# ashvardanian/StringZilla

Hardware: AMD Instinct MI355X
Metric: DP cell-updates/s (GCUPS) on 1M-pair Levenshtein batch (higher is better)
Workload: dtype u32 bit-vectors (u64 results)

## Files before the change

### stringzilla_amd/csrc/hip/device_common.hpp

```cpp
#pragma once
#include <hip/hip_runtime.h>
#include <stdint.h>

#include "kernels.h"

namespace szs_hip {

using u8 = uint8_t;
using u32 = uint32_t;
using u64 = uint64_t;
using i32 = int32_t;
using i64 = int64_t;

constexpr u32 wave_size_k = 64;

constexpr int device_slots_k = 64;
inline int device_slot() {
    int device = 0;
    if (hipGetDevice(&device) != hipSuccess) (void)hipGetLastError(), device = 0;
    return device < 0 || device >= device_slots_k ? 0 : device;
}
inline int cached(int const *slot) { return __atomic_load_n(slot, __ATOMIC_RELAXED); }
inline void remember(int *slot, int value) { __atomic_store_n(slot, value, __ATOMIC_RELAXED); }

__device__ __forceinline__ u32 wave_max_u32(u32 value) {
#pragma unroll
    for (int offset = 32; offset >= 1; offset >>= 1) {
        u32 const other = (u32)__shfl_xor((int)value, offset, 64);
        value = other > value ? other : value;
    }
    return value;
}

struct text_stream_t {
    u32 const *aligned_base;
    u32 byte_shift;
    u32 valid_dwords;

    __device__ __forceinline__ text_stream_t(u64 address, u32 length) {
        aligned_base = reinterpret_cast<u32 const *>(address & ~(u64)3);
        byte_shift = (u32)(address & 3);
        valid_dwords = length ? (byte_shift + length + 3) / 4 : 0;
    }

    __device__ __forceinline__ u32 raw(u32 dword_index) const {
        return dword_index < valid_dwords ? aligned_base[dword_index] : 0u;
    }

    __device__ __forceinline__ u32 raw_clamped(u32 dword_index) const {
        return aligned_base[dword_index < valid_dwords ? dword_index : valid_dwords - 1];
    }

    __device__ __forceinline__ u32 splice(u32 raw_low, u32 raw_high) const {
        return __builtin_amdgcn_alignbyte(raw_high, raw_low, byte_shift);
    }

    __device__ __forceinline__ static u32 symbol(u32 symbols, int step) { return (symbols >> (8 * step)) & 0xFFu; }
};

struct text_stream_backward_t {
    u32 const *aligned_base;
    u32 byte_shift;
    u32 valid_dwords;
    u32 top_dword;

    __device__ __forceinline__ text_stream_backward_t(u64 address, u32 length) {
        aligned_base = reinterpret_cast<u32 const *>(address & ~(u64)3);
        u64 const top = (address & 3) + (u64)length;
        byte_shift = (u32)(top & 3);
        valid_dwords = length ? (u32)((top + 3) / 4) : 0;
        top_dword = (u32)(top / 4);
    }

    __device__ __forceinline__ u32 raw(u32 back) const {
        u32 const dword_index = top_dword - back;
        return dword_index < valid_dwords ? aligned_base[dword_index] : 0u;
    }

    __device__ __forceinline__ u32 splice(u32 raw_high, u32 raw_low) const {
        return __builtin_amdgcn_alignbyte(raw_high, raw_low, byte_shift);
    }

    __device__ __forceinline__ static u32 symbol(u32 symbols, int step) { return (symbols >> (8 * (3 - step))) & 0xFFu; }
};

}
```

### stringzilla_amd/csrc/hip/lev_myers.hip

```cpp
#include "myers_core.hpp"

#define SZS_PAIR_RULE_FN __host__ __device__ static inline
#include "pair_rule.h"

#include <cstdlib>

namespace szs_hip {

#ifndef SZS_MYERS_PACK_QUERIES
#define SZS_MYERS_PACK_QUERIES 1
#endif
#ifndef SZS_MYERS_PAIR_RULES
#define SZS_MYERS_PAIR_RULES 1
#endif

#ifndef SZS_MYERS_SHORT_TEXT_DWORDS
#define SZS_MYERS_SHORT_TEXT_DWORDS 2
#endif


__device__ __forceinline__ u32 bits_in_word(u32 from, u32 to, int w) {
    u32 const low = from > 32u * w ? from : 32u * w, high = to < 32u * w + 32u ? to : 32u * w + 32u;
    if (low >= high) return 0u;
    return (high - low == 32u ? ~0u : (1u << (high - low)) - 1u) << (low - 32u * w);
}

template <int words_, int text_dwords_, bool runes_, bool paired_ = false>
__device__ __forceinline__ void myers_workgroup(u32 *peq, u32 *keys, szs_string_ref_t const query,
                                                szs_string_ref_t const *__restrict__ candidates, u32 candidates_count,
                                                u32 candidate_block, u64 *__restrict__ results, u64 results_row_stride,
                                                int symmetric, szs_ref_guard_t const &guard, u32 alphabet = 0,
                                                u32 *claimed_rows = nullptr, u32 blocks_here = 1, szs_string_ref_t const second = {}) {
    static_assert(!paired_ || !runes_, "query pairs are a byte-kernel shape");
    constexpr int rows = runes_ ? rune_slots_k : byte_rows_k;
    using layout = peq_layout<words_, rows>;
    if (guard.enabled && (!ref_is_current(guard, 0, query) || (paired_ && !ref_is_current(guard, 0, second)))) {
        if (threadIdx.x == 0) *guard.stale = guard.sequence;
        return;
    }
    u32 const first_length = query.length, second_length = paired_ ? second.length : 0u;
    u32 const query_length = paired_ ? first_length + second_length : first_length;
    u32 const used_rows = paired_ ? query_length + 2u : query_length;
    u32 const pad = 32u * words_ - used_rows;
    u32 const second_row = pad + first_length + 2u;

    for (int i = threadIdx.x; i < layout::total_dwords; i += 256) peq[i] = 0;
    if constexpr (runes_) {
        if (alphabet) {
            for (u32 i = threadIdx.x; i <= alphabet; i += 256) keys[i] = 0;
            if (threadIdx.x == 0) *claimed_rows = 0;
        }
        else
            for (int i = threadIdx.x; i < rune_slots_k; i += 256) keys[i] = rune_slot_empty_k;
    }
    __syncthreads();
    if (runes_ && alphabet) {
        u32 const *pattern = reinterpret_cast<u32 const *>(query.address);
        for (u32 i = threadIdx.x; i < query_length; i += 256) {
            u32 const id = pattern[i];
            if (atomicCAS(&keys[id], 0u, ~0u) == 0u) keys[id] = atomicAdd(claimed_rows, 1u) + 1;
        }
        __syncthreads();
        for (u32 i = threadIdx.x; i < query_length; i += 256) {
            u32 const position = pad + i;
            atomicOr(&peq[layout::dword_index((int)keys[pattern[i]], (int)(position >> 5))], 1u << (position & 31));
        }
    }
    else if constexpr (runes_) {
        u32 const *pattern = reinterpret_cast<u32 const *>(query.address);
        for (u32 i = threadIdx.x; i < query_length; i += 256) {
            u32 const rune = pattern[i];
            u32 slot = rune_slot_hash(rune);
            for (;;) {
                u32 const previous = atomicCAS(&keys[slot], rune_slot_empty_k, rune);
                if (previous == rune_slot_empty_k || previous == rune) break;
                slot = (slot + 1) & (rune_slots_k - 1);
            }
            u32 const position = pad + i;
            atomicOr(&peq[layout::dword_index((int)slot, (int)(position >> 5))], 1u << (position & 31));
        }
    }
    else {
        u8 const *pattern = reinterpret_cast<u8 const *>(query.address);
        for (u32 i = threadIdx.x; i < first_length; i += 256) {
            u32 const position = pad + i;
            atomicOr(&peq[layout::dword_index(pattern[i], (int)(position >> 5))], 1u << (position & 31));
        }
        if constexpr (paired_) {
            u8 const *above = reinterpret_cast<u8 const *>(second.address);
            for (u32 i = threadIdx.x; i < second_length; i += 256) {
                u32 const position = second_row + i;
                atomicOr(&peq[layout::dword_index(above[i], (int)(position >> 5))], 1u << (position & 31));
            }
        }
    }
    __syncthreads();
    pattern_pair_t<words_> boundary;
    if constexpr (paired_) {
#pragma unroll
        for (int w = 0; w < words_; ++w) {
            boundary.separators[w] = bits_in_word(second_row - 2u, second_row, w);
            boundary.tops[w] = first_length ? bits_in_word(second_row - 3u, second_row - 2u, w) : 0u;
        }
    }

#pragma unroll 1
    for (u32 block_step = 0; block_step < blocks_here; ++block_step) {
    u32 const candidate_slot = (candidate_block - block_step) * SZS_CANDIDATES_PER_WORKGROUP + threadIdx.x;
    bool live = candidate_slot < candidates_count;
    szs_string_ref_t candidate = {0, 0, 0};
    if (live) candidate = candidates[candidate_slot];
    if (live && guard.enabled && !ref_is_current(guard, 1, candidate)) {
        *guard.stale = guard.sequence;
        live = false;
    }
    if ((symmetric & SZS_LAYOUT_SYMMETRIC) && candidate.index > query.index) live = false;
    u32 const text_length = live ? candidate.length : 0;
    u32 const longest_in_wave = wave_max_u32(text_length);
    u32 const shortest_in_wave = ~wave_max_u32(live ? ~text_length : 0u);

    u32 vp[words_], vn[words_];
#pragma unroll
    for (int w = 0; w < words_; ++w) {
        vp[w] = bits_in_word(pad, 32u * words_, w) & ~(paired_ ? boundary.separators[w] : 0u);
        vn[w] = 0;
    }

    auto take = [&](u32 symbol) {
        u32 eq[words_];
        load_match_masks<words_, rows>(peq, !runes_ ? symbol : alphabet ? keys[symbol] : find_rune_slot(keys, symbol), eq);
        if constexpr (paired_) myers_column<words_>(vp, vn, eq, boundary);
        else myers_column<words_>(vp, vn, eq);
    };

    u32 column = 0;
    if constexpr (runes_) {
        u32 const *const runes = reinterpret_cast<u32 const *>(candidate.address);
        auto quad_at = [&](u32 index) -> uint4 {
            return index < text_length ? *reinterpret_cast<uint4 const *>(runes + index) : make_uint4(0, 0, 0, 0);
        };
        if (4 <= shortest_in_wave && longest_in_wave) {
            uint4 ahead = quad_at(0);
            for (; column + 4 <= shortest_in_wave; column += 4) {
                uint4 const now = ahead;
                ahead = quad_at(column + 4);
                take(now.x), take(now.y), take(now.z), take(now.w);
            }
        }
#pragma unroll 1
        for (; column < longest_in_wave; ++column)
            if (column < text_length) take(runes[column]);
    }
    else {
        u64 const safe_address = text_length ? candidate.address : first_length || !paired_ ? query.address : second.address;
        text_stream_t text(safe_address, text_length);
        if (!text_length) text.valid_dwords = query_length ? 1 : 0;
        u32 raw_low = text.raw(0);
        u32 dword = 0;
        constexpr u32 columns_per_iteration = 4 * text_dwords_;
#ifndef SZS_MYERS_CLAMPED_READS
#define SZS_MYERS_CLAMPED_READS(TEXT_DWORDS) ((TEXT_DWORDS) == 1)
#endif
        constexpr bool clamped_reads = SZS_MYERS_CLAMPED_READS(text_dwords_);
        if (columns_per_iteration <= shortest_in_wave && longest_in_wave && query_length) {
            u32 ahead[text_dwords_];
#pragma unroll
            for (int d = 0; d < text_dwords_; ++d) ahead[d] = clamped_reads ? text.raw_clamped(1 + d) : text.raw(1 + d);
            for (; column + columns_per_iteration <= shortest_in_wave;
                 column += columns_per_iteration, dword += text_dwords_) {
                u32 symbols[text_dwords_];
                symbols[0] = text.splice(raw_low, ahead[0]);
#pragma unroll
                for (int d = 1; d < text_dwords_; ++d) symbols[d] = text.splice(ahead[d - 1], ahead[d]);
                raw_low = ahead[text_dwords_ - 1];
#pragma unroll
                for (int d = 0; d < text_dwords_; ++d)
                    ahead[d] = clamped_reads ? text.raw_clamped(dword + text_dwords_ + 1 + d)
                                             : text.raw(dword + text_dwords_ + 1 + d);
#pragma unroll
                for (int step = 0; step < 4 * text_dwords_; ++step) take((symbols[step / 4] >> (8 * (step % 4))) & 0xFFu);
            }
        }
#ifndef SZS_MYERS_MID_LOOP
#define SZS_MYERS_MID_LOOP 0
#endif
        if constexpr (SZS_MYERS_MID_LOOP && text_dwords_ > 1) {
            if (column + 4 <= shortest_in_wave && longest_in_wave && query_length) {
                u32 ahead_one = text.raw(dword + 1);
#pragma unroll 1
                for (; column + 4 <= shortest_in_wave; column += 4, ++dword) {
                    u32 const symbols = text.splice(raw_low, ahead_one);
                    raw_low = ahead_one;
                    ahead_one = text.raw(dword + 2);
#pragma unroll
                    for (int step = 0; step < 4; ++step) take((symbols >> (8 * step)) & 0xFFu);
                }
            }
        }
        if (column < longest_in_wave) {
            u32 next = text.raw(dword + 1);
#pragma unroll 1
            for (; column < longest_in_wave; column += 4, ++dword) {
                u32 const after = text.raw(dword + 2);
                u32 const symbols = text.splice(raw_low, next);
                raw_low = next, next = after;
#pragma unroll
                for (int step = 0; step < 4; ++step)
                    if (column + step < text_length) take((symbols >> (8 * step)) & 0xFFu);
            }
        }
    }

    if (live && paired_) {
        u32 first = text_length, above = text_length;
#pragma unroll
        for (int w = 0; w < words_; ++w) {
            u32 const mine = bits_in_word(pad, pad + first_length, w), theirs = bits_in_word(second_row, 32u * words_, w);
            first += (u32)__builtin_popcount(vp[w] & mine) - (u32)__builtin_popcount(vn[w] & mine);
            above += (u32)__builtin_popcount(vp[w] & theirs) - (u32)__builtin_popcount(vn[w] & theirs);
        }
        bool const transposed = (symmetric & SZS_LAYOUT_TRANSPOSED) != 0;
        u64 const one = transposed ? candidate.index : query.index, two = transposed ? candidate.index : second.index;
        u64 const one_column = transposed ? query.index : candidate.index, two_column = transposed ? second.index : candidate.index;
        results[one * results_row_stride + one_column] = first;
        results[two * results_row_stride + two_column] = above;
    }
    else if (live) {
        u32 distance = text_length;
#pragma unroll
        for (int w = 0; w < words_; ++w) distance += (u32)__builtin_popcount(vp[w]) - (u32)__builtin_popcount(vn[w]);
        bool const transposed = (symmetric & SZS_LAYOUT_TRANSPOSED) != 0;
        u64 const row = transposed ? candidate.index : query.index, column = transposed ? query.index : candidate.index;
        results[row * results_row_stride + column] = distance;
        if ((symmetric & SZS_LAYOUT_SYMMETRIC) && candidate.index != query.index)
            results[column * results_row_stride + row] = distance;
    }
    }
}

#ifndef SZS_WORK_BLOCK_MAJOR
#define SZS_WORK_BLOCK_MAJOR 1
#endif
__device__ __forceinline__ void myers_work_item(u32 candidate_blocks, u32 &query_slot, u32 &candidate_block) {
#if SZS_WORK_BLOCK_MAJOR
    u32 const queries_count = gridDim.x / candidate_blocks;
    query_slot = blockIdx.x % queries_count;
    candidate_block = candidate_blocks - 1 - blockIdx.x / queries_count;
#else
    query_slot = blockIdx.x / candidate_blocks;
    candidate_block = candidate_blocks - 1 - blockIdx.x % candidate_blocks;
#endif
}

#ifndef SZS_MYERS_LONG_WAVES
#define SZS_MYERS_LONG_WAVES 2
#endif
template <int words_>
__global__ __launch_bounds__(256, SZS_MYERS_LONG_WAVES) void levenshtein_myers_long_kernel(szs_string_ref_t const *__restrict__ queries,
                                                                      szs_string_ref_t const *__restrict__ candidates,
                                                                      u32 candidates_count, u32 candidate_blocks,
                                                                      u64 *__restrict__ results, u64 results_row_stride,
                                                                      int symmetric, szs_ref_guard_t guard) {
    __shared__ __attribute__((aligned(16))) u32 peq[peq_layout<words_>::total_dwords];
    u32 query_slot, candidate_block;
    myers_work_item(candidate_blocks, query_slot, candidate_block);
    myers_workgroup<words_, 1, false>(peq, nullptr, queries[query_slot], candidates, candidates_count, candidate_block,
                                      results, results_row_stride, symmetric, guard);
}

__device__ __forceinline__ u64 fused_offset(void const *offsets, u32 wide, u64 index) {
    return wide ? static_cast<u64 const *>(offsets)[index] : (u64) static_cast<u32 const *>(offsets)[index];
}

__device__ __forceinline__ void fused_sort_side(szs_plan_side_t const &side, u32 is_query_side, u32 choose_rule, u32 sequence, u32 *ready,
                                                u32 second_ready, u32 withhold, szs_fused_side_report_t *report, u32 *histogram ,
                                                szs_string_ref_t *staged ) {
    constexpr u32 per_thread = SZS_FUSED_MOST_STRINGS / 256;
    u32 const tid = threadIdx.x, lane = tid & 63u, wave = tid >> 6, count = side.count;
    bool const one_pass = count <= SZS_FUSED_MOST_STRINGS;
    __shared__ u32 wave_bins[4], wave_longest[4], wave_status[4];
    __shared__ unsigned long long wave_symbols[4], wave_bands_systolic[4], wave_bands_chain[4], wave_squares[4];
    __shared__ u32 rule_words[256];

    u64 const began = wall_clock64();
    for (u32 bin = tid; bin < SZS_FUSED_BINS; bin += 256) histogram[bin] = 0;
    u64 from[per_thread], to[per_thread];
#pragma unroll
    for (u32 k = 0; k < per_thread; ++k) {
        u32 const i = tid + k * 256;
        from[k] = to[k] = 0;
        if (one_pass && i < count) from[k] = fused_offset(side.offsets, side.wide, i), to[k] = fused_offset(side.offsets, side.wide, (u64)i + 1);
    }
    __syncthreads();
    u32 bins[per_thread];
    u32 status = 0, longest = 0;
    u64 symbols = 0, bands_systolic = 0, bands_chain = 0, squares = 0;
    auto count_in = [&](u64 first, u64 last) -> u32 {
        if (last < first) return status |= SZS_PLAN_STATUS_DESCENDING, ~0u;
        if (last - first > 0xFFFFFFFFull) return status |= SZS_PLAN_STATUS_OVERFLOW, ~0u;
        u32 const length = (u32)(last - first);
        symbols += length, squares += (u64)length * length, longest = length > longest ? length : longest;
        bands_systolic += length ? (length + SZS_SYSTOLIC_BAND_ROWS - 1) / SZS_SYSTOLIC_BAND_ROWS : 1;
        bands_chain += length ? (length + SZS_MYERS_CHAIN_BAND_ROWS - 1) / SZS_MYERS_CHAIN_BAND_ROWS : 1;
        u32 const bin = length < SZS_FUSED_BINS - 1 ? length : SZS_FUSED_BINS - 1;
        atomicAdd(&histogram[bin], 1u);
        return bin;
    };
    if (one_pass) {
#pragma unroll
        for (u32 k = 0; k < per_thread; ++k) {
            bins[k] = ~0u;
            if (tid + k * 256 < count) bins[k] = count_in(from[k], to[k]);
        }
    }
    else {
#pragma unroll 1
        for (u32 first = 0; first < count; first += 1024) {
            u64 some_from[4], some_to[4];
#pragma unroll
            for (u32 k = 0; k < 4; ++k) {
                u32 const i = first + tid + k * 256;
                some_from[k] = some_to[k] = 0;
                if (i < count) some_from[k] = fused_offset(side.offsets, side.wide, i), some_to[k] = fused_offset(side.offsets, side.wide, (u64)i + 1);
            }
#pragma unroll
            for (u32 k = 0; k < 4; ++k)
                if (first + tid + k * 256 < count) (void)count_in(some_from[k], some_to[k]);
        }
    }
    if (tid == 0) report->ticks[0] = (u32)began, report->ticks[1] = (u32)(wall_clock64() - began);
#pragma unroll
    for (int offset = 32; offset >= 1; offset >>= 1) {
        status |= (u32)__shfl_xor((int)status, offset, 64);
        u32 const other = (u32)__shfl_xor((int)longest, offset, 64);
        longest = other > longest ? other : longest;
    }
    if (lane == 0) wave_status[wave] = status, wave_longest[wave] = longest;
    __syncthreads();
    u32 mine[4], sum = 0;
#pragma unroll
    for (u32 k = 0; k < 4; ++k) mine[k] = histogram[4 * tid + k], sum += mine[k];
    u32 inclusive = sum;
#pragma unroll
    for (int offset = 1; offset < 64; offset <<= 1) {
        u32 const other = (u32)__shfl_up((int)inclusive, offset, 64);
        if (lane >= (u32)offset) inclusive += other;
    }
    if (lane == 63) wave_bins[wave] = inclusive;
    __syncthreads();
    status = wave_status[0] | wave_status[1] | wave_status[2] | wave_status[3];
    longest = wave_longest[0];
#pragma unroll
    for (u32 w = 1; w < 4; ++w) longest = wave_longest[w] > longest ? wave_longest[w] : longest;
    u32 running = inclusive - sum;
    for (u32 w = 0; w < wave; ++w) running += wave_bins[w];
#pragma unroll
    for (u32 k = 0; k < 4; ++k) histogram[4 * tid + k] = running, running += mine[k];
    __syncthreads();
    if (tid == 0) report->ticks[2] = (u32)(wall_clock64() - began);
    u32 const blank = status || (is_query_side && longest > 32u * SZS_MYERS_SHORT_WORDS);
    if (one_pass) {
#pragma unroll
        for (u32 k = 0; k < per_thread; ++k) {
            u32 const i = tid + k * 256;
            if (i >= count) continue;
            szs_string_ref_t ref;
            ref.address = status ? side.base : side.base + from[k], ref.length = blank ? 0u : (u32)(to[k] - from[k]), ref.index = i;
            staged[status ? i : atomicAdd(&histogram[bins[k]], 1u)] = ref;
        }
        __syncthreads();
        for (u32 position = tid; position < count; position += 256) {
            szs_string_ref_t const ref = staged[position];
            side.ascending[position] = ref, side.descending[count - 1 - position] = ref;
        }
    }
    u32 const pair_slots = szs_pair_slots(count), pair_seconds = szs_pair_seconds(count);
    bool const choosing = choose_rule && one_pass && pair_seconds;
    if (choosing) {
        constexpr u32 strides = 256 / SZS_PAIR_RULE_CANDIDATES;
        u32 me = tid;
        asm volatile("" : "+v"(me));
        u32 const rule = szs_pair_rule_candidate(me % SZS_PAIR_RULE_CANDIDATES, pair_seconds);
        u32 words = 0;
        if (me < strides * SZS_PAIR_RULE_CANDIDATES) {
#pragma unroll 4
            for (u32 slot = me / SZS_PAIR_RULE_CANDIDATES; slot < pair_seconds; slot += strides)
                words += szs_pair_slot_words(staged[count - 1 - slot].length,
                                             staged[count - 1 - szs_pair_second_rank(rule, slot, pair_slots, pair_seconds)].length);
        }
        rule_words[me] = words;
    }
    if (!one_pass) {
#pragma unroll 1
        for (u32 first = 0; first < count; first += 1024) {
            u64 some_from[4], some_to[4];
#pragma unroll
            for (u32 k = 0; k < 4; ++k) {
                u32 const i = first + tid + k * 256;
                some_from[k] = some_to[k] = 0;
                if (i < count) some_from[k] = fused_offset(side.offsets, side.wide, i), some_to[k] = fused_offset(side.offsets, side.wide, (u64)i + 1);
            }
#pragma unroll
            for (u32 k = 0; k < 4; ++k) {
                u32 const i = first + tid + k * 256;
                if (i >= count) continue;
                u32 const length = status ? 0u : (u32)(some_to[k] - some_from[k]);
                szs_string_ref_t ref;
                ref.address = status ? side.base : side.base + some_from[k], ref.length = blank ? 0u : length, ref.index = i;
                u32 const position = status ? i : atomicAdd(&histogram[length < SZS_FUSED_BINS - 1 ? length : SZS_FUSED_BINS - 1], 1u);
                side.ascending[position] = ref, side.descending[count - 1 - position] = ref;
            }
        }
    }
    __syncthreads();
    if (tid == 0) report->ticks[3] = (u32)(wall_clock64() - began);
    u32 pairing = 0;
    if (choosing && wave == 0) {
        constexpr u32 strides = 256 / SZS_PAIR_RULE_CANDIDATES;
        u32 key = ~0u;
        if (lane < SZS_PAIR_RULE_CANDIDATES) {
            u32 total = 0;
#pragma unroll
            for (u32 k = 0; k < strides; ++k) total += rule_words[lane + k * SZS_PAIR_RULE_CANDIDATES];
            key = (total << 5) | lane;
        }
#pragma unroll
        for (int offset = 16; offset >= 1; offset >>= 1) {
            u32 const other = (u32)__shfl_xor((int)key, offset, 64);
            key = other < key ? other : key;
        }
        pairing = szs_pair_rule_candidate(key & 31u, pair_seconds);
    }
    if (tid == 0) {
        if (!withhold) {
            if (is_query_side)
                __hip_atomic_store(reinterpret_cast<u64 *>(ready), ((u64)pairing << 32) | sequence, __ATOMIC_RELEASE, __HIP_MEMORY_SCOPE_AGENT);
            else
                __hip_atomic_store(ready, sequence, __ATOMIC_RELEASE, __HIP_MEMORY_SCOPE_AGENT);
            if (second_ready) __hip_atomic_store(ready + 32, sequence, __ATOMIC_RELAXED, __HIP_MEMORY_SCOPE_AGENT);
        }
        report->ticks[4] = (u32)(wall_clock64() - began);
    }
#pragma unroll
    for (int offset = 32; offset >= 1; offset >>= 1) {
        symbols += ((u64)(u32)__shfl_xor((int)(u32)(symbols >> 32), offset, 64) << 32) | (u32)__shfl_xor((int)(u32)symbols, offset, 64);
        squares += ((u64)(u32)__shfl_xor((int)(u32)(squares >> 32), offset, 64) << 32) | (u32)__shfl_xor((int)(u32)squares, offset, 64);
        bands_systolic += ((u64)(u32)__shfl_xor((int)(u32)(bands_systolic >> 32), offset, 64) << 32) | (u32)__shfl_xor((int)(u32)bands_systolic, offset, 64);
        bands_chain += ((u64)(u32)__shfl_xor((int)(u32)(bands_chain >> 32), offset, 64) << 32) | (u32)__shfl_xor((int)(u32)bands_chain, offset, 64);
    }
    if (lane == 0) wave_symbols[wave] = symbols, wave_bands_systolic[wave] = bands_systolic, wave_bands_chain[wave] = bands_chain, wave_squares[wave] = squares;
    if (tid <= SZS_PLAN_RANK_SAMPLES) {
        u32 const rank = (u32)((u64)tid * (count ? count - 1 : 0) / SZS_PLAN_RANK_SAMPLES);
        report->rank_lengths[tid] = status || !count ? 0u : one_pass ? staged[rank].length : side.ascending[rank].length;
    }
    __syncthreads();
    if (tid == 0) {
        report->status = status, report->blank = blank, report->pairing = pairing;
        report->stats.count = count, report->stats.longest = longest;
        report->stats.symbols = wave_symbols[0] + wave_symbols[1] + wave_symbols[2] + wave_symbols[3];
        report->stats.bands_systolic = wave_bands_systolic[0] + wave_bands_systolic[1] + wave_bands_systolic[2] + wave_bands_systolic[3];
        report->stats.bands_chain = wave_bands_chain[0] + wave_bands_chain[1] + wave_bands_chain[2] + wave_bands_chain[3];
        report->squares = wave_squares[0] + wave_squares[1] + wave_squares[2] + wave_squares[3];
        report->sequence = sequence;
    }
}

__device__ __forceinline__ bool fused_prologue(szs_fused_plan_t const &plan, u32 *scratch, u32 &pairing) {
    __shared__ __attribute__((aligned(16))) szs_string_ref_t staged[SZS_FUSED_MOST_STRINGS];
    for (u32 s = 0; s < (plan.symmetric ? 1u : 2u); ++s)
        if (blockIdx.x == s % gridDim.x) {
            fused_sort_side(plan.side[s], s == 0, SZS_MYERS_PAIR_RULES && SZS_MYERS_PACK_QUERIES && s == 0 && !plan.symmetric && plan.blocks_per_group == 1,
                            plan.sequence, plan.ready + 32 * s, plan.symmetric, plan.withhold, plan.report + s, scratch, staged);
            __syncthreads();
        }
    __shared__ u32 unpublished[2], published_high[2];
    if (threadIdx.x < 2) {
        u32 polls = 0;
        u64 word;
        bool published;
        while (!(published = (u32)(word = __hip_atomic_load(reinterpret_cast<u64 const *>(plan.ready + 32 * threadIdx.x), __ATOMIC_RELAXED,
                                                             __HIP_MEMORY_SCOPE_AGENT)) == plan.sequence) &&
               ++polls < plan.poll_budget)
            __builtin_amdgcn_s_sleep(8);
        unpublished[threadIdx.x] = !published, published_high[threadIdx.x] = (u32)(word >> 32);
    }
    __syncthreads();
    pairing = (u32)__builtin_amdgcn_readfirstlane((int)published_high[0]);
    if (unpublished[0] | unpublished[1]) {
        if (threadIdx.x == 0) __hip_atomic_store(plan.gave_up, plan.sequence, __ATOMIC_RELAXED, __HIP_MEMORY_SCOPE_SYSTEM);
        return false;
    }
    return true;
}

#ifndef SZS_MYERS_SHORT_WAVES
#define SZS_MYERS_SHORT_WAVES 1
#endif
constexpr u32 szs_myers_pair_words_k = SZS_PAIR_WORDS_MOST;
template <bool runes_, bool merged_, bool fused_ = false>
__device__ __forceinline__ void myers_short_body(
    szs_string_ref_t const *__restrict__ queries, szs_string_ref_t const *__restrict__ candidates, u32 candidates_count,
    u32 candidate_blocks, u64 *__restrict__ results, u64 results_row_stride, int symmetric, szs_ref_guard_t guard, u32 alphabet,
    u32 blocks_per_group, szs_fused_plan_t const *fused = nullptr) {
    constexpr bool pairs = fused_ && !merged_ && SZS_MYERS_PACK_QUERIES;
    __shared__ __attribute__((aligned(16))) u32 peq[peq_layout<pairs ? szs_myers_pair_words_k : 8, runes_ ? rune_slots_k : byte_rows_k>::total_dwords];
    u32 pairing = 0;
    if constexpr (fused_) {
        static_assert(peq_layout<8, byte_rows_k>::total_dwords >= SZS_FUSED_BINS, "the sort's histogram borrows the masks' LDS");
        if (!fused_prologue(*fused, peq, pairing)) return;
    }
    __shared__ u32 slot_keys[runes_ ? rune_slots_k : 1];
    __shared__ u32 claimed_rows;
    extern __shared__ u32 rows_of_ids[];
    u32 *const keys = runes_ && alphabet ? rows_of_ids : slot_keys;
    u32 query_slot, candidate_group;
    myers_work_item(candidate_blocks, query_slot, candidate_group);
    u32 const all_blocks = (candidates_count + SZS_CANDIDATES_PER_WORKGROUP - 1) / SZS_CANDIDATES_PER_WORKGROUP;
    u32 const first_block = merged_ ? candidate_group * blocks_per_group : candidate_group;
    u32 const blocks_here = !merged_ ? 1u : all_blocks - first_block < blocks_per_group ? all_blocks - first_block : blocks_per_group;
    u32 const candidate_block = first_block + blocks_here - 1;
    szs_string_ref_t query = queries[query_slot];
    if constexpr (fused_) {
        query.address = ((u64)(u32)__builtin_amdgcn_readfirstlane((int)(u32)(query.address >> 32)) << 32) |
                        (u32)__builtin_amdgcn_readfirstlane((int)(u32)query.address);
// ... 1232 lines not shown
```

### stringzilla_amd/csrc/hip/myers_core.hpp

```cpp
#pragma once
#include "device_common.hpp"

namespace szs_hip {

constexpr int byte_rows_k = 256;
constexpr int rune_slots_k = 512;
constexpr u32 rune_slot_empty_k = ~0u;

template <int words_, int rows_ = byte_rows_k>
struct peq_layout {
    static constexpr int chunk_words = words_ >= 3 ? 4 : words_;
    static constexpr int chunks = (words_ + chunk_words - 1) / chunk_words;
    static constexpr int total_dwords = chunks * rows_ * chunk_words;
    __device__ static constexpr int dword_index(int row, int w) {
        return ((w / chunk_words) * rows_ + row) * chunk_words + (w % chunk_words);
    }
};

__device__ __forceinline__ u32 rune_slot_hash(u32 rune) { return (rune * 2654435761u) >> 23; }
__device__ __forceinline__ u32 find_rune_slot(u32 const *keys, u32 rune) {
    u32 slot = rune_slot_hash(rune);
    for (;;) {
        u32 const key = keys[slot];
        if (key == rune || key == rune_slot_empty_k) return slot;
        slot = (slot + 1) & (rune_slots_k - 1);
    }
}

template <int words_, int rows_>
__device__ __forceinline__ void load_match_masks(u32 const *peq, u32 symbol, u32 (&eq)[words_]) {
    using layout = peq_layout<words_, rows_>;
    if constexpr (layout::chunk_words == 4) {
        uint4 const *rows = reinterpret_cast<uint4 const *>(peq);
#pragma unroll
        for (int chunk = 0; chunk < layout::chunks; ++chunk) {
            uint4 const row = rows[chunk * rows_ + symbol];
            if (chunk * 4 + 0 < words_) eq[chunk * 4 + 0] = row.x;
            if (chunk * 4 + 1 < words_) eq[chunk * 4 + 1] = row.y;
            if (chunk * 4 + 2 < words_) eq[chunk * 4 + 2] = row.z;
            if (chunk * 4 + 3 < words_) eq[chunk * 4 + 3] = row.w;
        }
    }
    else if constexpr (layout::chunk_words == 2) {
        uint2 const row = reinterpret_cast<uint2 const *>(peq)[symbol];
        eq[0] = row.x, eq[1] = row.y;
    }
    else { eq[0] = peq[symbol]; }
}

__device__ __forceinline__ bool ref_is_current(szs_ref_guard_t const &guard, int side, szs_string_ref_t const &ref) {
    if (ref.index >= guard.side[side].count) return false;
    u64 from, to;
    if (guard.side[side].wide) {
        u64 const *offsets = static_cast<u64 const *>(guard.side[side].offsets);
        from = offsets[ref.index], to = offsets[(u64)ref.index + 1];
    }
    else {
        u32 const *offsets = static_cast<u32 const *>(guard.side[side].offsets);
        from = offsets[ref.index], to = offsets[(u64)ref.index + 1];
    }
    return to >= from && to - from == ref.length && guard.side[side].base + from == ref.address;
}

struct single_pattern_t {
    __device__ static constexpr u32 separator(int) { return 0; }
    __device__ static constexpr u32 top(int) { return 0; }
};

template <int words_>
struct pattern_pair_t {
    u32 separators[words_], tops[words_];
    __device__ u32 separator(int w) const { return separators[w]; }
    __device__ u32 top(int w) const { return tops[w]; }
};

template <int words_, typename boundary_t = single_pattern_t, bool materialise_ = true>
__device__ __forceinline__ void myers_column(u32 (&vp)[words_], u32 (&vn)[words_], u32 const (&eq)[words_],
                                             boundary_t const &boundary = {}) {
    u32 carry = 0, hp_below = 0, hn_below = 0;
#pragma unroll
    for (int w = 0; w < words_; ++w) {
        u32 xv = eq[w] | vn[w];
        if constexpr (!std::is_same<boundary_t, single_pattern_t>::value)
            asm("v_bitop3_b32 %0, %1, %2, %3 bitop3:0xfe" : "=v"(xv) : "v"(eq[w]), "v"(vn[w]), "v"(boundary.separator(w)));
        u32 carry_out;
        u32 const sum = __builtin_addc(eq[w] & vp[w], vp[w], carry, &carry_out);
        carry = carry_out;
        u32 const d0 = (sum ^ vp[w]) | eq[w];
        u32 const hp = vn[w] | ~(d0 | vp[w]);
        u32 const hn = vp[w] & d0 & ~boundary.top(w);
        u32 const hp_shifted = w == 0 ? ((hp << 1) | 1u) : __builtin_amdgcn_alignbit(hp, hp_below, 31);
        u32 const hn_shifted = w == 0 ? (hn << 1) : __builtin_amdgcn_alignbit(hn, hn_below, 31);
        hp_below = hp, hn_below = hn;
        vp[w] = hn_shifted | ~(xv | hp_shifted);
        vn[w] = hp_shifted & xv & ~boundary.separator(w);
        if constexpr (materialise_ && words_ > 1) asm("" : "+v"(vp[w]), "+v"(vn[w]));
    }
}

template <int words_>
__device__ __forceinline__ u32 myers_infix_column(u32 (&vp)[words_], u32 (&vn)[words_], u32 const (&eq)[words_]) {
    u32 carry = 0, hp_below = 0, hn_below = 0;
#pragma unroll
    for (int w = 0; w < words_; ++w) {
        u32 const xv = eq[w] | vn[w];
        u32 carry_out;
        u32 const sum = __builtin_addc(eq[w] & vp[w], vp[w], carry, &carry_out);
        carry = carry_out;
        u32 const d0 = (sum ^ vp[w]) | eq[w];
        u32 const hp = vn[w] | ~(d0 | vp[w]);
        u32 const hn = vp[w] & d0;
        u32 const hp_shifted = w == 0 ? (hp << 1) : __builtin_amdgcn_alignbit(hp, hp_below, 31);
        u32 const hn_shifted = w == 0 ? (hn << 1) : __builtin_amdgcn_alignbit(hn, hn_below, 31);
        hp_below = hp, hn_below = hn;
        vp[w] = hn_shifted | ~(xv | hp_shifted);
        vn[w] = hp_shifted & xv;
        if constexpr (words_ > 1) asm("" : "+v"(vp[w]), "+v"(vn[w]));
    }
    return (hp_below >> 31) | ((hn_below >> 31) << 1);
}

template <int words_>
__device__ __forceinline__ u32 myers_prefix_column(u32 (&vp)[words_], u32 (&vn)[words_], u32 const (&eq)[words_]) {
    u32 carry = 0, hp_below = 0, hn_below = 0;
#pragma unroll
    for (int w = 0; w < words_; ++w) {
        u32 const xv = eq[w] | vn[w];
        u32 carry_out;
        u32 const sum = __builtin_addc(eq[w] & vp[w], vp[w], carry, &carry_out);
        carry = carry_out;
        u32 const d0 = (sum ^ vp[w]) | eq[w];
        u32 const hp = vn[w] | ~(d0 | vp[w]);
        u32 const hn = vp[w] & d0;
        u32 const hp_shifted = w == 0 ? ((hp << 1) | 1u) : __builtin_amdgcn_alignbit(hp, hp_below, 31);
        u32 const hn_shifted = w == 0 ? (hn << 1) : __builtin_amdgcn_alignbit(hn, hn_below, 31);
        hp_below = hp, hn_below = hn;
        vp[w] = hn_shifted | ~(xv | hp_shifted);
        vn[w] = hp_shifted & xv;
        if constexpr (words_ > 1) asm("" : "+v"(vp[w]), "+v"(vn[w]));
    }
    return (hp_below >> 31) | ((hn_below >> 31) << 1);
}

template <int words_>
__device__ __forceinline__ u32 myers_strip_column(u32 (&vp)[words_], u32 (&vn)[words_], u32 const (&eq)[words_], u32 hp_in,
                                                  u32 hn_in) {
    u32 carry = 0, hp_below = 0, hn_below = 0;
#pragma unroll
    for (int w = 0; w < words_; ++w) {
        u32 const xv = eq[w] | vn[w];
        u32 const eq_in = w == 0 ? (eq[w] | hn_in) : eq[w];
        u32 carry_out;
        u32 const sum = __builtin_addc(eq_in & vp[w], vp[w], carry, &carry_out);
        carry = carry_out;
        u32 const d0 = (sum ^ vp[w]) | eq_in;
        u32 const hp = vn[w] | ~(d0 | vp[w]);
        u32 const hn = vp[w] & d0;
        u32 const hp_shifted = w == 0 ? ((hp << 1) | hp_in) : __builtin_amdgcn_alignbit(hp, hp_below, 31);
        u32 const hn_shifted = w == 0 ? ((hn << 1) | hn_in) : __builtin_amdgcn_alignbit(hn, hn_below, 31);
        hp_below = hp, hn_below = hn;
        vp[w] = hn_shifted | ~(xv | hp_shifted);
        vn[w] = hp_shifted & xv;
    }
    return (hp_below >> 31) | ((hn_below >> 31) << 1);
}

}
```

Measured before the change: 100,700.

## Add software-pipelined Myers column loop and global address-space text loads

Marks the text stream pointers as global address space (address_space(1)) by default, so the compiler can emit global loads instead of flat loads. It also adds an optional column-pipelined path that prefetches the next symbol's match-vector chunks from the peq table while the current column computes. The prefetch is placed with sched_barriers through a new per-word hook in myers_column. The pipeline path is off by default (SZS_MYERS_COLUMN_PIPELINE=0), so only the global-load typing takes effect, and it adds complexity plus register pressure when enabled.

```diff
diff --git a/stringzilla_amd/csrc/hip/device_common.hpp b/stringzilla_amd/csrc/hip/device_common.hpp
--- a/stringzilla_amd/csrc/hip/device_common.hpp
+++ b/stringzilla_amd/csrc/hip/device_common.hpp
@@ -32,13 +32,22 @@
     return value;
 }
 
+#ifndef SZS_TEXT_GLOBAL_LOADS
+#define SZS_TEXT_GLOBAL_LOADS 1
+#endif
+#if SZS_TEXT_GLOBAL_LOADS
+typedef u32 const __attribute__((address_space(1))) *text_dwords_t;
+#else
+typedef u32 const *text_dwords_t;
+#endif
+
 struct text_stream_t {
-    u32 const *aligned_base;
+    text_dwords_t aligned_base;
     u32 byte_shift;
     u32 valid_dwords;
 
     __device__ __forceinline__ text_stream_t(u64 address, u32 length) {
-        aligned_base = reinterpret_cast<u32 const *>(address & ~(u64)3);
+        aligned_base = reinterpret_cast<text_dwords_t>(address & ~(u64)3);
         byte_shift = (u32)(address & 3);
         valid_dwords = length ? (byte_shift + length + 3) / 4 : 0;
     }
@@ -59,13 +68,13 @@
 };
 
 struct text_stream_backward_t {
-    u32 const *aligned_base;
+    text_dwords_t aligned_base;
     u32 byte_shift;
     u32 valid_dwords;
     u32 top_dword;
 
     __device__ __forceinline__ text_stream_backward_t(u64 address, u32 length) {
-        aligned_base = reinterpret_cast<u32 const *>(address & ~(u64)3);
+        aligned_base = reinterpret_cast<text_dwords_t>(address & ~(u64)3);
         u64 const top = (address & 3) + (u64)length;
         byte_shift = (u32)(top & 3);
         valid_dwords = length ? (u32)((top + 3) / 4) : 0;
diff --git a/stringzilla_amd/csrc/hip/lev_myers.hip b/stringzilla_amd/csrc/hip/lev_myers.hip
--- a/stringzilla_amd/csrc/hip/lev_myers.hip
+++ b/stringzilla_amd/csrc/hip/lev_myers.hip
@@ -16,6 +16,10 @@
 
 #ifndef SZS_MYERS_SHORT_TEXT_DWORDS
 #define SZS_MYERS_SHORT_TEXT_DWORDS 2
+#endif
+
+#ifndef SZS_MYERS_COLUMN_PIPELINE
+#define SZS_MYERS_COLUMN_PIPELINE 0
 #endif
 
 
@@ -162,7 +166,64 @@
 #define SZS_MYERS_CLAMPED_READS(TEXT_DWORDS) ((TEXT_DWORDS) == 1)
 #endif
         constexpr bool clamped_reads = SZS_MYERS_CLAMPED_READS(text_dwords_);
+        if constexpr (SZS_MYERS_COLUMN_PIPELINE && text_dwords_ > 1) {
         if (columns_per_iteration <= shortest_in_wave && longest_in_wave && query_length) {
+            constexpr int chunk_words = layout::chunk_words, chunks = layout::chunks;
+            constexpr int held_chunks = SZS_MYERS_COLUMN_PIPELINE == 2 ? chunks : 1;
+            constexpr int read_behind_word = held_chunks == 1 && words_ > 8 ? chunk_words - 1 : -1;
+            u32 symbols[text_dwords_], ahead[text_dwords_];
+#pragma unroll
+            for (int d = 0; d < text_dwords_; ++d) ahead[d] = text.raw_clamped(1 + d);
+            symbols[0] = text.splice(raw_low, ahead[0]);
+#pragma unroll
+            for (int d = 1; d < text_dwords_; ++d) symbols[d] = text.splice(ahead[d - 1], ahead[d]);
+            raw_low = ahead[text_dwords_ - 1];
+#pragma unroll
+            for (int d = 0; d < text_dwords_; ++d) ahead[d] = text.raw_clamped(text_dwords_ + 1 + d);
+            u32 held[held_chunks][chunk_words];
+#pragma unroll
+            for (int chunk = 0; chunk < held_chunks; ++chunk) load_match_chunk<words_, rows>(peq, symbols[0] & 0xFFu, chunk, held[chunk]);
+            for (; column + columns_per_iteration <= shortest_in_wave; column += columns_per_iteration, dword += text_dwords_) {
+#pragma unroll
+                for (int step = 0; step < (int)columns_per_iteration; ++step) {
+                    u32 const symbol = text_stream_t::symbol(symbols[step / 4], step % 4);
+                    u32 eq[words_];
+#pragma unroll
+                    for (int chunk = 0; chunk < chunks; ++chunk) {
+                        u32 part[chunk_words];
+                        if (chunk >= held_chunks) load_match_chunk<words_, rows>(peq, symbol, chunk, part);
+#pragma unroll
+                        for (int k = 0; k < chunk_words; ++k)
+                            if (chunk * chunk_words + k < words_) eq[chunk * chunk_words + k] = chunk < held_chunks ? held[chunk][k] : part[k];
+                    }
+                    if (step + 1 == (int)columns_per_iteration) {
+                        __builtin_amdgcn_sched_barrier(0);
+                        symbols[0] = text.splice(raw_low, ahead[0]);
+#pragma unroll
+                        for (int d = 1; d < text_dwords_; ++d) symbols[d] = text.splice(ahead[d - 1], ahead[d]);
+                        asm volatile("v_mov_b32 %0, %1" : "=v"(raw_low) : "v"(ahead[text_dwords_ - 1]));
+#pragma unroll
+                        for (int d = 0; d < text_dwords_; ++d) asm volatile("" : "+v"(symbols[d])::"memory");
+#pragma unroll
+                        for (int d = 0; d < text_dwords_; ++d) ahead[d] = text.raw_clamped(dword + 2 * text_dwords_ + 1 + d);
+                    }
+                    u32 const following = text_stream_t::symbol(symbols[(step + 1) % (int)columns_per_iteration / 4], (step + 1) % 4);
+                    auto read_ahead = [&](int behind_word) {
+                        if (behind_word != read_behind_word) return;
+                        if (behind_word >= 0) __builtin_amdgcn_sched_barrier(0);
+#pragma unroll
+                        for (int chunk = 0; chunk < held_chunks; ++chunk) load_match_chunk<words_, rows>(peq, following, chunk, held[chunk]);
+                        __builtin_amdgcn_sched_barrier(0);
+                    };
+                    read_ahead(-1);
+                    if constexpr (paired_) myers_column<words_>(vp, vn, eq, boundary, read_ahead);
+                    else myers_column<words_>(vp, vn, eq, single_pattern_t {}, read_ahead);
+                }
+            }
+            raw_low = text.raw_clamped(dword);
+        }
+        }
+        else if (columns_per_iteration <= shortest_in_wave && longest_in_wave && query_length) {
             u32 ahead[text_dwords_];
 #pragma unroll
             for (int d = 0; d < text_dwords_; ++d) ahead[d] = clamped_reads ? text.raw_clamped(1 + d) : text.raw(1 + d);
@@ -213,13 +274,20 @@
 
     if (live && paired_) {
         u32 first = text_length, above = text_length;
+        u32 first_row = pad, first_end = pad + first_length, above_row = second_row;
+        if constexpr (SZS_MYERS_COLUMN_PIPELINE != 0) asm volatile("" : "+s"(first_row), "+s"(first_end), "+s"(above_row));
 #pragma unroll
         for (int w = 0; w < words_; ++w) {
-            u32 const mine = bits_in_word(pad, pad + first_length, w), theirs = bits_in_word(second_row, 32u * words_, w);
+            u32 const mine = bits_in_word(first_row, first_end, w), theirs = bits_in_word(above_row, 32u * words_, w);
             first += (u32)__builtin_popcount(vp[w] & mine) - (u32)__builtin_popcount(vn[w] & mine);
             above += (u32)__builtin_popcount(vp[w] & theirs) - (u32)__builtin_popcount(vn[w] & theirs);
         }
         bool const transposed = (symmetric & SZS_LAYOUT_TRANSPOSED) != 0;
+        if constexpr (SZS_MYERS_COLUMN_PIPELINE != 0) {
+            u32 slot = candidate_slot;
+            asm volatile("" : "+v"(slot));
+            candidate.index = candidates[slot].index;
+        }
         u64 const one = transposed ? candidate.index : query.index, two = transposed ? candidate.index : second.index;
         u64 const one_column = transposed ? query.index : candidate.index, two_column = transposed ? second.index : candidate.index;
         results[one * results_row_stride + one_column] = first;
diff --git a/stringzilla_amd/csrc/hip/myers_core.hpp b/stringzilla_amd/csrc/hip/myers_core.hpp
--- a/stringzilla_amd/csrc/hip/myers_core.hpp
+++ b/stringzilla_amd/csrc/hip/myers_core.hpp
@@ -48,6 +48,20 @@
     else { eq[0] = peq[symbol]; }
 }
 
+template <int words_, int rows_>
+__device__ __forceinline__ void load_match_chunk(u32 const *peq, u32 symbol, int chunk, u32 (&part)[peq_layout<words_, rows_>::chunk_words]) {
+    using layout = peq_layout<words_, rows_>;
+    if constexpr (layout::chunk_words == 4) {
+        uint4 const row = reinterpret_cast<uint4 const *>(peq)[chunk * rows_ + symbol];
+        part[0] = row.x, part[1] = row.y, part[2] = row.z, part[3] = row.w;
+    }
+    else if constexpr (layout::chunk_words == 2) {
+        uint2 const row = reinterpret_cast<uint2 const *>(peq)[symbol];
+        part[0] = row.x, part[1] = row.y;
+    }
+    else { part[0] = peq[symbol]; }
+}
+
 __device__ __forceinline__ bool ref_is_current(szs_ref_guard_t const &guard, int side, szs_string_ref_t const &ref) {
     if (ref.index >= guard.side[side].count) return false;
     u64 from, to;
@@ -74,9 +88,13 @@
     __device__ u32 top(int w) const { return tops[w]; }
 };
 
-template <int words_, typename boundary_t = single_pattern_t, bool materialise_ = true>
+struct no_word_hook_t {
+    __device__ void operator()(int) const {}
+};
+
+template <int words_, typename boundary_t = single_pattern_t, bool materialise_ = true, typename word_hook_t = no_word_hook_t>
 __device__ __forceinline__ void myers_column(u32 (&vp)[words_], u32 (&vn)[words_], u32 const (&eq)[words_],
-                                             boundary_t const &boundary = {}) {
+                                             boundary_t const &boundary = {}, word_hook_t const &after_word = {}) {
     u32 carry = 0, hp_below = 0, hn_below = 0;
 #pragma unroll
     for (int w = 0; w < words_; ++w) {
@@ -95,6 +113,7 @@
         vp[w] = hn_shifted | ~(xv | hp_shifted);
         vn[w] = hp_shifted & xv & ~boundary.separator(w);
         if constexpr (materialise_ && words_ > 1) asm("" : "+v"(vp[w]), "+v"(vn[w]));
+        after_word(w);
     }
 }
 
```

Measured after the change: 99760. No clear change (-0.9%).
